# RomanBresson/KAGNN

Measured on AMD Instinct MI355X. Metric: edges/sec KAN-GIN fwd+bwd, hidden=64 grid=5, 1M-node synthetic; HBM % peak, higher is better.
Workload: dtype f32 (fp16 hi/lo split operands, fp32 accumulate)

## Files before the change

kagnn_amd/csrc/fused_calls.hip:

```cpp
#include "host.h"
#include <mutex>

using namespace kagnn;

namespace {
struct GraphSide {
    const int32_t* rowptr; const int32_t* col; const int32_t* hub_seg; int64_t num_hub_seg; int32_t hub_threshold; float self_scale;
};
struct KanChain {
    int64_t N; int32_t L; const int32_t* widths;
    const float* const* bw; const float* const* sw; const float* const* sc;
    const float* const* acts; const void* const* pack_fwd; const void* const* pack_dx;
    const float* knots; int32_t G, K, mode;
};
struct LayerIn {
    const void* x; int32_t x_dtype; int64_t ldx; const float* in_col_scale; const float* in_col_shift; float* col_mean; float* col_m2;
};
struct LayerGrads {
    const float* gy; int64_t ldgy; void* gx; int32_t gx_dtype; int64_t ldgx; int32_t bf16_gather; const float* gx_addend; int64_t ld_addend;
    float* const* g_bw; float* const* g_sw; float* const* g_sc;
};

struct GineStage {
    const float* x; int64_t ldx; const float* ea; int64_t lde; const int32_t* perm;
    float* g_ea; int64_t ldge;
    int accumulate_g_ea = 0;
    int prepacked = 0;
};
struct BnStage { const float* y; int64_t ldy; const float* weight; const float* mean; const float* rstd; float* g_weight; float* g_bias; };
struct StatsOut { const float* y; int64_t ldy; const float* mean; const float* rstd; float* sums; };
struct DwPiece { unsigned char* base; DwDefer* defer; };

struct LayerLayout {
    size_t fwd_hub_bytes, fwd_scratch, fwd_scratch_bytes, fwd_fix, fwd_fix_bytes, fwd_total;
    size_t bwd_hub_bytes, dw, dw_bytes, g[2], bwd_total;
    size_t bn, bn_ws_bytes, bn_tab, bn_bytes, stats, stats_bytes, bwd_total_all;
    size_t dw_piece[8], dw_piece_bytes[8], dw_pieces_bytes;
    int wmax;
};

void layer_layout_optional(LayerLayout& y, int64_t N, int out, int f0, int64_t num_hub_seg_t) {
    y.bn = y.bwd_total;
    y.bn_ws_bytes = out ? bn_ws_bytes(N, out) : 0;
    y.bn_tab = y.bn + al256z(y.bn_ws_bytes);
    y.bn_bytes = out ? al256z(y.bn_ws_bytes) + al256z(4 * (size_t)((out + 63) & ~63) * sizeof(float)) : 0;
    y.stats = y.bn + y.bn_bytes;
    y.stats_bytes = f0 ? al256z(bn_stats_fold_bytes(aggregate_stats_rows(N, f0, num_hub_seg_t), f0)) : 0;
    y.bwd_total_all = y.stats + y.stats_bytes;
}

int layer_layout(int64_t N, int32_t L, const int32_t* widths, int32_t G, int32_t K, int32_t mode, int64_t num_hub_seg,
                 int64_t num_hub_seg_t, LayerLayout& y) {
    static const char fn[] = "kagnn_gin_kan_layer_workspace_bytes";
    size_t fw = 0, dw = 0;
    y.wmax = 0;
    for (int l = 0; l < L; ++l) {
        int rc = check_kan_dims(fn, widths[l], widths[l + 1], G, K, mode);
        if (rc) return rc;
        size_t b = 0;
        rc = (l == L - 1 ? kagnn_kan_fwd_moments_workspace_bytes : kagnn_kan_fwd_workspace_bytes)(N, widths[l], widths[l + 1], G, K, mode, &b);
        if (rc) return rc;
        fw = b > fw ? b : fw;
        rc = kagnn_kan_bwd_weight_workspace_bytes(N, widths[l], widths[l + 1], G, K, mode, &b); if (rc) return rc;
        dw = b > dw ? b : dw;
        y.dw_piece_bytes[l] = al256z(b);
        y.wmax = widths[l] > y.wmax ? widths[l] : y.wmax;
    }
    y.dw_pieces_bytes = 0;
    for (int l = L - 1; l >= 0; --l) { y.dw_piece[l] = y.dw_pieces_bytes; y.dw_pieces_bytes += y.dw_piece_bytes[l]; }
    y.fwd_hub_bytes = al256z(aggregate_bf16_ws_bytes(num_hub_seg, widths[0]));
    y.fwd_scratch = y.fwd_hub_bytes;
    y.fwd_fix = y.fwd_scratch + al256z(fw);
    y.fwd_total = y.fwd_fix + al256z(widths[0] <= 32 ? kan_sparse_fwd_agg_ws_bytes(num_hub_seg, widths[0], widths[1]) : 0) + 256;
    y.fwd_scratch_bytes = y.fwd_total - y.fwd_scratch;
    y.fwd_fix_bytes = y.fwd_total - y.fwd_fix;
    y.bwd_hub_bytes = al256z(aggregate_bf16_ws_bytes(num_hub_seg_t, widths[0]));
    y.dw = y.bwd_hub_bytes;
    y.dw_bytes = al256z(dw);
    const size_t g_bytes = al256z((size_t)N * y.wmax * sizeof(float));
    y.g[0] = y.dw + y.dw_bytes;
    y.g[1] = y.g[0] + g_bytes;
    y.bwd_total = y.g[1] + g_bytes + 256;
    layer_layout_optional(y, N, 0, 0, 0);
    return KAGNN_OK;
}

int layer_fwd_impl(const GraphSide& gr, const KanChain& c, const LayerIn& in, const GineStage* gine, void* workspace,
                   size_t workspace_bytes, void* stream, const char* fn) {
    (void)fn;
    const int64_t N = c.N;
    const int32_t L = c.L, G = c.G, K = c.K, mode = c.mode;
    const int32_t* widths = c.widths;
    float* const* acts = const_cast<float* const*>(c.acts);
    void* const* pack_fwd = const_cast<void* const*>(c.pack_fwd);
    void* const* pack_dx = const_cast<void* const*>(c.pack_dx);
    KAGNN_CHECK_ARG(N >= 0 && L >= 1 && L <= 8 && widths && c.bw && c.sw && acts && pack_fwd && pack_dx, "bad argument");
    KAGNN_CHECK_ARG((in.in_col_scale == nullptr) == (in.in_col_shift == nullptr), "in_col_scale and in_col_shift must both be given or both be null");
    KAGNN_CHECK_ARG(!in.in_col_scale || in.x_dtype == KAGNN_DTYPE_F32, "the column affine of the gathered matrix needs fp32 rows");
    KAGNN_CHECK_ARG((in.col_mean == nullptr) == (in.col_m2 == nullptr), "col_mean and col_m2 must both be given or both be null");
    LayerLayout lay;
    int rc = layer_layout(N, L, widths, G, K, mode, gr.num_hub_seg, 0, lay);
    if (rc) return rc;
    KAGNN_CHECK_ARG(workspace && workspace_bytes >= lay.fwd_total, "workspace too small (kagnn_gin_kan_layer_workspace_bytes)");
    if (N == 0) return KAGNN_OK;
    unsigned char* ws = static_cast<unsigned char*>(workspace);
    const char* fuse_e = getenv("KAGNN_FUSE_AGG");
    const bool fuse_env = fuse_e != nullptr && atoi(fuse_e) != 0;
    const bool fuse = fuse_env && !gine && !in.in_col_scale && in.x_dtype == KAGNN_DTYPE_F32 && mode == KAGNN_PREC_SPLIT && !(L == 1 && in.col_mean) &&
                      use_sparse_fwd(widths[0], widths[1], G, K, mode) &&
                      kan_sparse_fwd_agg_ok(static_cast<const float*>(in.x), in.ldx, N, widths[0], widths[1], G, K);
    if (gine)
        rc = kagnn_aggregate_gine(static_cast<const float*>(in.x), in.ldx, gine->ea, gine->lde, acts[0], widths[0], gr.rowptr, gr.col, gine->perm, N,
                                  widths[0], gr.self_scale, stream);
    else if (fuse)
        rc = KAGNN_OK;
    else if (in.x_dtype == KAGNN_DTYPE_BF16)
        rc = kagnn_aggregate_sum_bf16(in.x, in.ldx, acts[0], widths[0], KAGNN_DTYPE_F32, gr.rowptr, gr.col, nullptr, N, widths[0], gr.self_scale,
                                      nullptr, nullptr, nullptr, 0, gr.hub_seg, gr.num_hub_seg, gr.hub_threshold, ws, lay.fwd_hub_bytes, stream);
    else if (in.in_col_scale)
        rc = kagnn_aggregate_sum_affine(static_cast<const float*>(in.x), in.ldx, acts[0], widths[0], gr.rowptr, gr.col, N, widths[0], gr.self_scale,
                                        in.in_col_scale, in.in_col_shift, gr.hub_seg, gr.num_hub_seg, gr.hub_threshold, nullptr, 0, ws,
                                        lay.fwd_hub_bytes, stream);
    else
        rc = kagnn_aggregate_sum(static_cast<const float*>(in.x), in.ldx, acts[0], widths[0], gr.rowptr, gr.col, nullptr, N, widths[0],
                                 gr.self_scale, nullptr, nullptr, nullptr, 0, gr.hub_seg, gr.num_hub_seg, gr.hub_threshold, ws, lay.fwd_hub_bytes,
                                 stream);
    if (rc) return rc;
    const bool prepacked = gine && gine->prepacked;
    bool batched = L >= 2 && !prepacked;
    int in_[8], out_[8];
    for (int l = 0; l < L; ++l) {
        in_[l] = widths[l]; out_[l] = widths[l + 1];
        batched = batched && use_split_dx(in_[l], out_[l], G, K, mode) && use_sparse_fwd(in_[l], out_[l], G, K, mode) &&
                  kan_fused_pack_ok(in_[l], out_[l], G + K);
    }
    if (batched) {
        rc = kagnn_kan_pack_batch(L, c.bw, c.sw, c.sc, in_, out_, G, K, mode, pack_fwd, pack_dx, stream);
        if (rc) return rc;
    } else if (!prepacked) {
        for (int l = 0; l < L; ++l) {
            rc = kagnn_kan_pack(c.bw[l], c.sw[l], c.sc ? c.sc[l] : nullptr, in_[l], out_[l], G, K, mode, pack_fwd[l], pack_dx[l], stream);
            if (rc) return rc;
        }
    }
    for (int l = 0; l < L; ++l) {
        if (l == 0 && fuse) {
            KAGNN_STAGE_AS("kagnn_kan_linear_fwd+aggregate_sum (one kernel)", stream);
            rc = kan_sparse_fwd_agg(static_cast<const float*>(in.x), in.ldx, N, gr.rowptr, gr.col, gr.hub_seg, gr.num_hub_seg, gr.hub_threshold,
                                    gr.self_scale, c.knots, in_[0], out_[0], G, K, pack_fwd[0], acts[0], in_[0], acts[1], out_[0],
                                    ws + lay.fwd_fix, lay.fwd_fix_bytes, as_stream(stream));
            if (rc) return rc;
            continue;
        }
        if (l == L - 1 && in.col_mean)
            rc = kagnn_kan_linear_fwd_moments(acts[l], in_[l], N, c.knots, in_[l], out_[l], G, K, mode, pack_fwd[l], acts[l + 1],
                                              out_[l], in.col_mean, in.col_m2, ws + lay.fwd_scratch, lay.fwd_scratch_bytes, stream);
        else
            rc = kagnn_kan_linear_fwd(acts[l], in_[l], N, c.knots, in_[l], out_[l], G, K, mode, pack_fwd[l], acts[l + 1], out_[l],
                                      ws + lay.fwd_scratch, lay.fwd_scratch_bytes, stream);
        if (rc) return rc;
    }
    return KAGNN_OK;
}

struct BwdSide { hipStream_t stream = nullptr; hipEvent_t fork = nullptr, join = nullptr; };
constexpr int kBwdSideMaxDevices = 64;
std::mutex g_bwd_side_mu;
BwdSide g_bwd_side[kBwdSideMaxDevices];

class BwdFork {
    std::unique_lock<std::mutex> lk_;
    BwdSide* s_ = nullptr;
    hipStream_t caller_ = nullptr;
    bool forked_ = false, recorded_ = false;
public:
    BwdFork() = default;
    BwdFork(const BwdFork&) = delete;
    BwdFork& operator=(const BwdFork&) = delete;
    int prepare(hipStream_t caller) {
        int dev = 0;
        KAGNN_HIP(hipGetDevice(&dev));
        if (dev < 0 || dev >= kBwdSideMaxDevices) return fail(KAGNN_ERR_UNSUPPORTED, "%s: device index out of range", "layer_bwd");
        lk_ = std::unique_lock<std::mutex>(g_bwd_side_mu);
        BwdSide& s = g_bwd_side[dev];
        if (!s.stream) KAGNN_HIP(hipStreamCreateWithFlags(&s.stream, hipStreamNonBlocking));
        if (!s.fork) KAGNN_HIP(hipEventCreateWithFlags(&s.fork, hipEventDisableTiming));
        if (!s.join) KAGNN_HIP(hipEventCreateWithFlags(&s.join, hipEventDisableTiming));
        s_ = &s; caller_ = caller;
        return KAGNN_OK;
    }
    int fork() {
        KAGNN_HIP(hipEventRecord(s_->fork, caller_));
        KAGNN_HIP(hipStreamWaitEvent(s_->stream, s_->fork, 0));
        forked_ = true;
        return KAGNN_OK;
    }
    hipStream_t side() const { return s_->stream; }
    int side_done(hipEvent_t* ev) {
        KAGNN_HIP(hipEventRecord(s_->join, s_->stream));
        recorded_ = true;
        *ev = s_->join;
        return KAGNN_OK;
    }
    void joined() { forked_ = false; }
    int join() {
        if (!forked_) return KAGNN_OK;
        forked_ = false;
        if (!recorded_) KAGNN_HIP(hipEventRecord(s_->join, s_->stream));
        KAGNN_HIP(hipStreamWaitEvent(caller_, s_->join, 0));
        return KAGNN_OK;
    }
    ~BwdFork() { (void)join(); }
};

constexpr int kAggCorunHeadPct = 35;
bool dw_corun_ok(int in, int out, int G, int K, int mode) {
    return use_split_dw(in, out, G, K, mode) && !g_half_products && K == 3 && G + K <= 8 && in > 32 && in <= 64 && out <= 64;
}

int layer_bwd_impl(const GraphSide& gr, const KanChain& c, const LayerGrads& io, const BnStage* bn, const float* bn_sums_in,
                   const StatsOut* so, const GineStage* gine, const DwPiece* piece, void* workspace, size_t workspace_bytes, void* stream,
                   const char* fn) {
    const int64_t N = c.N;
    const int32_t L = c.L, G = c.G, K = c.K, mode = c.mode;
    const int32_t* widths = c.widths;
    const float* const* acts = c.acts;
    void* const gx = io.gx;
    KAGNN_CHECK_ARG(N >= 0 && L >= 1 && L <= 8 && widths && c.sw && acts && c.pack_dx && io.g_sw, "bad argument");
    KAGNN_CHECK_ARG(!io.gx_addend || (gx && io.gx_dtype == KAGNN_DTYPE_F32 && !io.bf16_gather && io.ld_addend >= widths[0]),
                    "gx_addend needs an fp32 gx and fp32 gather operands");
    LayerLayout lay;
    int rc = layer_layout(N, L, widths, G, K, mode, 0, gr.num_hub_seg, lay);
    if (rc) return rc;
    layer_layout_optional(lay, N, bn ? widths[L] : 0, so ? widths[0] : 0, gr.num_hub_seg);
    KAGNN_CHECK_ARG(!so || (so->y && so->mean && so->rstd && so->sums && so->ldy >= widths[0] && gx && io.gx_dtype == KAGNN_DTYPE_F32 && !io.bf16_gather),
                    "the previous norm's statistics need its input, mean, rstd and an fp32 gx");
    KAGNN_CHECK_ARG(!bn_sums_in || bn, "bn_sums belongs to the BatchNorm stage");
    if (!(workspace && workspace_bytes >= lay.bwd_total_all))
        return fail(KAGNN_ERR_ARG, bn ? "%s: workspace too small (kagnn_gin_kan_layer_workspace_bytes + kagnn_gin_kan_layer_bwd_bn_workspace_bytes)"
                                      : "%s: workspace too small (kagnn_gin_kan_layer_workspace_bytes)", fn);
    if (N == 0) return KAGNN_OK;
    unsigned char* ws = static_cast<unsigned char*>(workspace);
    const int wmax = lay.wmax;
    unsigned char* gbuf[2] = {ws + lay.g[0], ws + lay.g[1]};
    auto dw_on = [&](void* st, int l, const float* g, long ldg) {
        unsigned char* area = piece ? piece->base + lay.dw_piece[l] : ws + lay.dw;
        const size_t bytes = piece ? lay.dw_piece_bytes[l] : lay.dw_bytes;
        return kan_linear_bwd_weight(acts[l], widths[l], nullptr, g, ldg, N, c.knots, widths[l], widths[l + 1], G, K, mode, c.sw[l],
                                     c.sc ? c.sc[l] : nullptr, io.g_bw ? io.g_bw[l] : nullptr, io.g_sw[l], io.g_sc ? io.g_sc[l] : nullptr,
                                     area, bytes, st, piece ? piece->defer : nullptr);
    };
    BwdFork side;
    struct { int l; const float* g; long ldg; } deferred[2];
    int n_deferred = 0;
    bool overlap = false;
    if (gx && !gine && !piece && !so && !io.bf16_gather && io.gx_dtype == KAGNN_DTYPE_F32 && dw_corun_ok(widths[0], widths[1], G, K, mode)) {
        const char* env = getenv("KAGNN_BWD_OVERLAP");
        const AggArgs probe{reinterpret_cast<const float*>(gbuf[0]), widths[0], static_cast<float*>(gx), io.ldgx, gr.rowptr, gr.col, nullptr, N,
                            widths[0], gr.self_scale, nullptr, nullptr, nullptr, 0, 0x7fffffff, io.gx_addend, io.ld_addend};
        const bool gx_in_ws = static_cast<unsigned char*>(gx) + (size_t)N * io.ldgx * sizeof(float) > ws &&
                              static_cast<unsigned char*>(gx) < ws + workspace_bytes;
        overlap = (env == nullptr || atoi(env) != 0) && io.ldgx >= widths[0] && (!io.gx_addend || io.ld_addend >= widths[0]) && !gx_in_ws &&
                  aggregate_corun_ok(probe);
        if (overlap) {
            hipStreamCaptureStatus cap = hipStreamCaptureStatusNone;
            if (hipStreamIsCapturing(as_stream(stream), &cap) != hipSuccess) { (void)hipGetLastError(); overlap = false; }
            else overlap = cap == hipStreamCaptureStatusNone;
        }
        if (overlap) { rc = side.prepare(as_stream(stream)); if (rc) return rc; }
    }
    auto dw = [&](int l, const float* g, long ldg) {
        const bool alive = l == 0 || (l == L - 1 && !bn);
        if (overlap && alive && dw_corun_ok(widths[l], widths[l + 1], G, K, mode)) {
            deferred[n_deferred++] = {l, g, ldg};
            return (int)KAGNN_OK;
        }
        return dw_on(stream, l, g, ldg);
    };
    const float* g = io.gy;
    long ldg = io.ldgy;
    int cur = 0;
    bool gh0_bf16 = false;
    bool bn_in_dx = false;
    BnBack bnb{};
    if (bn) {
        const int out = widths[L], ldt = (out + 63) & ~63;
        KAGNN_CHECK_ARG(bn->y && bn->mean && bn->rstd && bn->ldy >= out && N >= 2, "bad BatchNorm stage");
        unsigned char* bws = ws + lay.bn;
        float* tab = reinterpret_cast<float*>(ws + lay.bn_tab);
        bnb = BnBack{bn->y, (long)bn->ldy, tab, ldt, reinterpret_cast<float*>(gbuf[1]), (long)out};
        const int in = widths[L - 1];
        bn_in_dx = mode == KAGNN_PREC_SPLIT && use_split_dx(in, out, G, K, mode) && out <= wmax && !(L == 1 && (gx == nullptr || io.bf16_gather)) &&
                   fits32(N, ldg) && kan_split_dx_bn_ok(ldg, in, out, G, K, bnb, g);
        if (bn_in_dx && bn_sums_in) {
            KAGNN_STAGE_AS("kagnn_batchnorm_bwd statistics given (in ..._layer_bwd_bn)", stream);
            rc = bn_bwd_stats_given(bn_sums_in, N, out, bn->weight, bn->mean, bn->rstd, bn->g_weight, bn->g_bias, tab, ldt, as_stream(stream));
            if (rc) return rc;
        } else if (bn_in_dx) {
            KAGNN_STAGE_AS("kagnn_batchnorm_bwd statistics (in ..._layer_bwd_bn)", stream);
            rc = bn_bwd_stats(bn->y, bn->ldy, g, ldg, N, out, bn->weight, bn->mean, bn->rstd, bn->g_weight, bn->g_bias, tab, ldt, bws,
                              lay.bn_ws_bytes, as_stream(stream));
            if (rc) return rc;
        } else {
            if (out > wmax) return fail(KAGNN_ERR_UNSUPPORTED, "%s: a BatchNorm stage wider than every layer input is not covered", fn);
            KAGNN_STAGE_AS("kagnn_batchnorm_bwd", stream);
            rc = bn_bwd(bn->y, bn->ldy, g, ldg, N, out, bn->weight, bn->mean, bn->rstd, 1, 0.0f, 0ULL, reinterpret_cast<float*>(gbuf[1]), out,
                        bn->g_weight, bn->g_bias, bws, lay.bn_ws_bytes, as_stream(stream));
            if (rc) return rc;
            g = reinterpret_cast<const float*>(gbuf[1]); ldg = out;
        }
    }
    for (int l = L - 1; l >= 0; --l) {
        const int in = widths[l], out = widths[l + 1];
        const bool fused_bn = bn_in_dx && l == L - 1;
        if (fused_bn) {
            {
                KAGNN_STAGE_AS("kagnn_kan_linear_bwd_input", stream);
                rc = kan_split_dx_bn(acts[l], in, g, ldg, N, c.knots, in, out, G, K, c.pack_dx[l], reinterpret_cast<float*>(gbuf[0]), in, bnb,
                                     as_stream(stream));
            }
            if (rc) return rc;
            rc = dw(l, bnb.gy_out, bnb.ldo);
            if (rc) return rc;
            if (l == 0 && gx == nullptr) break;
            g = reinterpret_cast<const float*>(gbuf[0]); ldg = in; cur = 1;
            continue;
        }
        rc = dw(l, g, ldg);
        if (rc) return rc;
        if (l == 0 && gx == nullptr) break;
        const bool b16 = l == 0 && io.bf16_gather && mode == KAGNN_PREC_SPLIT && K == 3 && G + K <= 8 && out <= 128 && in % 8 == 0 &&
                         in <= 512  &&
                         use_split_dx(in, out, G, K, mode);
        rc = kagnn_kan_linear_bwd_input(acts[l], in, g, ldg, N, c.knots, in, out, G, K, mode, c.pack_dx[l], gbuf[cur], in,
                                        b16 ? KAGNN_DTYPE_BF16 : KAGNN_DTYPE_F32, stream);
        if (rc) return rc;
        g = reinterpret_cast<const float*>(gbuf[cur]); ldg = in; cur ^= 1;
        gh0_bf16 = b16;
    }
    if (gx == nullptr) return KAGNN_OK;
    const int f0 = widths[0];
    if (overlap) {
        rc = side.fork();
        if (rc) return rc;
        for (int k = 0; k < n_deferred; ++k) {
            rc = dw_on(side.side(), deferred[k].l, deferred[k].g, deferred[k].ldg);
            if (rc) return rc;
        }
        const AggArgs a{g, ldg, static_cast<float*>(gx), io.ldgx, gr.rowptr, gr.col, nullptr, N, f0, gr.self_scale, nullptr, nullptr, nullptr,
                        0, gr.hub_threshold > 0 ? gr.hub_threshold : 0x7fffffff, io.gx_addend, io.ld_addend};
        AggCorun corun{kAggCorunHeadPct * n_deferred, nullptr};
        rc = side.side_done(&corun.side_done);
        if (rc) return rc;
        KAGNN_STAGE_AS("kagnn_aggregate_sum", stream);
        rc = aggregate_sum(a, gr.hub_seg, gr.num_hub_seg, reinterpret_cast<float*>(ws), lay.bwd_hub_bytes, as_stream(stream), &corun);
        if (rc) return rc;
        side.joined();
        return KAGNN_OK;
    }
    if (gine)
        return gine_bwd(gine->x, gine->ldx, gine->ea, gine->lde, g, ldg, static_cast<float*>(gx), io.ldgx, gine->g_ea, gine->ldge,
                        gr.rowptr, gr.col, gine->perm, N, f0, gr.self_scale, as_stream(stream), gine->accumulate_g_ea);
    if (gh0_bf16 || io.gx_dtype == KAGNN_DTYPE_BF16) {
        const void* src = g;
        if (!gh0_bf16) {
            rc = kagnn_rows_to_bf16(g, ldg, gbuf[cur], f0, N, f0, stream);
            if (rc) return rc;
            src = gbuf[cur];
        }
        return kagnn_aggregate_sum_bf16(src, f0, gx, io.ldgx, io.gx_dtype, gr.rowptr, gr.col, nullptr, N, f0, gr.self_scale, nullptr, nullptr,
                                        nullptr, 0, gr.hub_seg, gr.num_hub_seg, gr.hub_threshold, ws, lay.bwd_hub_bytes, stream);
    }
    if (so) {
        AggArgs a{g, ldg, static_cast<float*>(gx), io.ldgx, gr.rowptr, gr.col, nullptr, N, f0, gr.self_scale, nullptr, nullptr, nullptr,
                  0, gr.hub_threshold > 0 ? gr.hub_threshold : 0x7fffffff, io.gx_addend, io.ld_addend};
        float* partial = reinterpret_cast<float*>(ws + lay.stats);
        a.st_y = so->y; a.st_ldy = so->ldy; a.st_mean = so->mean; a.st_rstd = so->rstd; a.st_partial = partial;
        KAGNN_CHECK_ARG(ldg >= f0 && io.ldgx >= f0 && (!io.gx_addend || io.ld_addend >= f0), "leading dimension smaller than num_feat");
        if (!aggregate_stats_ok(a)) return fail(KAGNN_ERR_UNSUPPORTED, "%s: the previous norm's statistics need 17..256 input features in 16-byte aligned fp32 rows", fn);
        {
            KAGNN_STAGE_AS("kagnn_aggregate_sum", stream);
            rc = aggregate_sum(a, gr.hub_seg, gr.num_hub_seg, reinterpret_cast<float*>(ws), lay.bwd_hub_bytes, as_stream(stream));
            if (rc) return rc;
        }
        KAGNN_STAGE_AS("kagnn_batchnorm_bwd statistics fold", stream);
        const bool hubs = gr.num_hub_seg > 0 && gr.hub_seg != nullptr && gr.hub_threshold > 0;
        return bn_sums_from_partials(partial, aggregate_stats_rows(N, f0, hubs ? gr.num_hub_seg : 0), f0, so->sums, as_stream(stream));
    }
    return kagnn_aggregate_sum_add(g, ldg, static_cast<float*>(gx), io.ldgx, gr.rowptr, gr.col, nullptr, N, f0, gr.self_scale, nullptr,
                                   nullptr, nullptr, 0, gr.hub_seg, gr.num_hub_seg, gr.hub_threshold, io.gx_addend, io.ld_addend, ws,
                                   lay.bwd_hub_bytes, stream);
}

struct StackLayout {
    LayerLayout layer;
    size_t fwd_layer_bytes, bn_ws, bn_ws_bytes, moments, fwd_total;
    size_t bwd_layer_bytes, pp[2], arena, arena_conv_bytes, arena_bytes, bwd_total;
};

int stack_layout(int64_t N, int32_t nconv, int32_t L, const int32_t* widths, int32_t G, int32_t K, int32_t mode, StackLayout& s) {
    int rc = layer_layout(N, L, widths, G, K, mode, 0, 0, s.layer);
    if (rc) return rc;
    layer_layout_optional(s.layer, N, widths[L], 0, 0);
    s.fwd_layer_bytes = al256z(s.layer.fwd_total);
    s.bn_ws = s.fwd_layer_bytes;
    s.bn_ws_bytes = bn_ws_bytes(N, widths[L]);
    s.moments = s.bn_ws + al256z(s.bn_ws_bytes);
    s.fwd_total = s.moments + al256z(2 * (size_t)widths[L] * sizeof(float)) + 256;
    s.bwd_layer_bytes = al256z(s.layer.bwd_total_all);
    const size_t g_bytes = al256z((size_t)N * widths[0] * sizeof(float));
    s.pp[0] = s.bwd_layer_bytes;
    s.pp[1] = s.pp[0] + g_bytes;
    s.arena = s.pp[1] + g_bytes;
    s.arena_conv_bytes = nconv * L <= kDwDeferMax ? s.layer.dw_pieces_bytes : 0;
    s.arena_bytes = s.arena_conv_bytes * (size_t)nconv;
    s.bwd_total = s.arena + s.arena_bytes + 256;
    return KAGNN_OK;
}

int stack_fwd_impl(const float* x, int64_t ldx, const float* edge_attr, int64_t lde, int64_t N, const int32_t* rowptr,
                   const int32_t* col, const int32_t* perm, const float* self_scale, int32_t nconv,
                   int32_t L, const int32_t* widths, const float* const* bw, const float* const* sw,
                   const float* const* sc, const float* knots, int32_t G, int32_t K, int32_t mode,
                   float* const* acts, void* const* pack_fwd, void* const* pack_dx,
                   const float* const* bn_weight, const float* const* bn_bias, float* const* running_mean,
                   float* const* running_var, const float* momentum, const float* eps,
                   float* const* h, float* const* save_mean, float* const* save_rstd,
                   void* workspace, size_t workspace_bytes, void* stream, bool prepacked) {
    static const char fn[] = "kagnn_gine_kan_stack_fwd";
    ModeScope mode_scope_(mode);
    KAGNN_CHECK_ARG_AS(fn, nconv >= 1 && L >= 1 && L <= 8 && widths && self_scale && bw && sw && acts && pack_fwd && pack_dx && bn_weight && bn_bias &&
                       momentum && eps && h && save_mean && save_rstd, "null array");
    KAGNN_CHECK_ARG_AS(fn, widths[0] == widths[L] && N >= 2, "hidden -> hidden chains, at least two rows (batch statistics)");
    StackLayout lay;
    int rc = stack_layout(N, nconv, L, widths, G, K, mode, lay);
    if (rc) return rc;
    KAGNN_CHECK_ARG_AS(fn, workspace && workspace_bytes >= lay.fwd_total, "workspace too small (kagnn_gine_kan_stack_workspace_bytes)");
    unsigned char* ws = static_cast<unsigned char*>(workspace);
    float* mom = reinterpret_cast<float*>(ws + lay.moments);
    const int H = widths[L];
    int in_[16], out_[16];
    bool batch = nconv * L <= 16;
    for (int k = 0; k < nconv * L && batch; ++k) {
        in_[k] = widths[k % L]; out_[k] = widths[k % L + 1];
        batch = use_split_dx(in_[k], out_[k], G, K, mode) && use_sparse_fwd(in_[k], out_[k], G, K, mode) && kan_fused_pack_ok(in_[k], out_[k], G + K);
    }
    if (batch && !prepacked) { rc = kagnn_kan_pack_batch(nconv * L, bw, sw, sc, in_, out_, G, K, mode, pack_fwd, pack_dx, stream); if (rc) return rc; }
    const float* in = x;
    int64_t ldin = ldx;
    for (int i = 0; i < nconv; ++i) {
        GineStage gs{in, ldin, edge_attr, lde, perm, nullptr, 0};
        gs.prepacked = batch ? 1 : 0;
        const GraphSide gr{.rowptr = rowptr, .col = col, .self_scale = self_scale[i]};
        const KanChain c{.N = N, .L = L, .widths = widths, .bw = bw + i * L, .sw = sw + i * L, .sc = sc ? sc + i * L : nullptr,
                         .acts = acts + i * (L + 1), .pack_fwd = pack_fwd + i * L, .pack_dx = pack_dx + i * L, .knots = knots, .G = G, .K = K,
                         .mode = mode};
        const LayerIn li{.x = in, .x_dtype = KAGNN_DTYPE_F32, .ldx = ldin, .col_mean = mom,
                         .col_m2 = mom + H};
        rc = layer_fwd_impl(gr, c, li, &gs, ws, lay.fwd_layer_bytes, stream, fn);
        if (rc) return rc;
        rc = kagnn_batchnorm_fwd(acts[i * (L + 1) + L], H, N, H, bn_weight[i], bn_bias[i], running_mean ? running_mean[i] : nullptr,
                                 running_var ? running_var[i] : nullptr, momentum[i], eps[i], 1, mom, mom + H, 0.0f, 0ULL, h[i], H,
                                 save_mean[i], save_rstd[i], ws + lay.bn_ws, lay.bn_ws_bytes, stream);
        if (rc) return rc;
        in = h[i]; ldin = H;
    }
    return KAGNN_OK;
}
}

#pragma GCC visibility push(default)
extern "C" {

int kagnn_gin_kan_layer_workspace_bytes(int64_t N, int32_t L, const int32_t* widths, int32_t G, int32_t K, int32_t mode,
                                        int64_t num_hub_seg, int64_t num_hub_seg_t, size_t* fwd_bytes, size_t* bwd_bytes) {
    ModeScope mode_scope_(mode);
    KAGNN_CHECK_ARG(N >= 0 && L >= 1 && L <= 8 && widths && fwd_bytes && bwd_bytes, "bad argument");
    LayerLayout lay;
    int rc = layer_layout(N, L, widths, G, K, mode, num_hub_seg, num_hub_seg_t, lay);
    if (rc) return rc;
    *fwd_bytes = lay.fwd_total;
    *bwd_bytes = lay.bwd_total;
    return KAGNN_OK;
}

int kagnn_gin_kan_layer_fwd(const void* x, int32_t x_dtype, int64_t ldx, int64_t N, const int32_t* rowptr, const int32_t* col,
                            const int32_t* hub_seg, int64_t num_hub_seg, int32_t hub_threshold, float self_scale,
                            int32_t L, const int32_t* widths, const float* const* bw, const float* const* sw,
                            const float* const* sc, const float* knots, int32_t G, int32_t K, int32_t mode,
                            float* const* acts, void* const* pack_fwd, void* const* pack_dx, float* col_mean,
                            float* col_m2, void* workspace, size_t workspace_bytes, void* stream) {
    ModeScope mode_scope_(mode);
    const GraphSide gr{.rowptr = rowptr, .col = col, .hub_seg = hub_seg, .num_hub_seg = num_hub_seg, .hub_threshold = hub_threshold,
                       .self_scale = self_scale};
    const KanChain c{.N = N, .L = L, .widths = widths, .bw = bw, .sw = sw, .sc = sc, .acts = acts, .pack_fwd = pack_fwd, .pack_dx = pack_dx,
                     .knots = knots, .G = G, .K = K, .mode = mode};
    const LayerIn in{.x = x, .x_dtype = x_dtype, .ldx = ldx, .col_mean = col_mean, .col_m2 = col_m2};
    return layer_fwd_impl(gr, c, in, nullptr, workspace, workspace_bytes, stream, __func__);
}

int kagnn_gin_kan_layer_fwd_affine(const float* x, int64_t ldx, int64_t N, const int32_t* rowptr, const int32_t* col,
                                   const int32_t* hub_seg, int64_t num_hub_seg, int32_t hub_threshold, float self_scale,
                                   const float* in_col_scale, const float* in_col_shift,
                                   int32_t L, const int32_t* widths, const float* const* bw, const float* const* sw,
                                   const float* const* sc, const float* knots, int32_t G, int32_t K, int32_t mode,
                                   float* const* acts, void* const* pack_fwd, void* const* pack_dx, float* col_mean,
                                   float* col_m2, void* workspace, size_t workspace_bytes, void* stream) {
    ModeScope mode_scope_(mode);
    const GraphSide gr{.rowptr = rowptr, .col = col, .hub_seg = hub_seg, .num_hub_seg = num_hub_seg, .hub_threshold = hub_threshold,
                       .self_scale = self_scale};
    const KanChain c{.N = N, .L = L, .widths = widths, .bw = bw, .sw = sw, .sc = sc, .acts = acts, .pack_fwd = pack_fwd, .pack_dx = pack_dx,
                     .knots = knots, .G = G, .K = K, .mode = mode};
    const LayerIn in{.x = x, .x_dtype = KAGNN_DTYPE_F32, .ldx = ldx, .in_col_scale = in_col_scale, .in_col_shift = in_col_shift,
                     .col_mean = col_mean, .col_m2 = col_m2};
    return layer_fwd_impl(gr, c, in, nullptr, workspace, workspace_bytes, stream, __func__);
}

int kagnn_gin_kan_layer_bwd_add(const float* gy, int64_t ldgy, int64_t N, const int32_t* rowptr_t, const int32_t* col_t,
                                const int32_t* hub_seg_t, int64_t num_hub_seg_t, int32_t hub_threshold, float self_scale,
                                int32_t L, const int32_t* widths, const float* const* sw, const float* const* sc,
                                const float* knots, int32_t G, int32_t K, int32_t mode, const float* const* acts,
                                const void* const* pack_dx, void* gx, int32_t gx_dtype, int64_t ldgx, int32_t bf16_gather,
                                const float* gx_addend, int64_t ld_addend,
                                float* const* g_bw, float* const* g_sw, float* const* g_sc, void* workspace,
                                size_t workspace_bytes, void* stream) {
    ModeScope mode_scope_(mode);
    const GraphSide gr{.rowptr = rowptr_t, .col = col_t, .hub_seg = hub_seg_t, .num_hub_seg = num_hub_seg_t, .hub_threshold = hub_threshold,
                       .self_scale = self_scale};
    const KanChain c{.N = N, .L = L, .widths = widths, .sw = sw, .sc = sc, .acts = acts, .pack_dx = pack_dx,
                     .knots = knots, .G = G, .K = K, .mode = mode};
    const LayerGrads io{.gy = gy, .ldgy = ldgy, .gx = gx, .gx_dtype = gx_dtype, .ldgx = ldgx, .bf16_gather = bf16_gather, .gx_addend = gx_addend,
                        .ld_addend = ld_addend, .g_bw = g_bw, .g_sw = g_sw, .g_sc = g_sc};
    return layer_bwd_impl(gr, c, io, nullptr, nullptr, nullptr, nullptr, nullptr, workspace, workspace_bytes, stream, __func__);
}

int kagnn_gin_kan_layer_bwd_bn_workspace_bytes(int64_t N, int32_t out, size_t* bytes) {
    KAGNN_CHECK_ARG(N >= 0 && out >= 1 && bytes, "bad argument");
    LayerLayout lay{};
    layer_layout_optional(lay, N, out, 0, 0);
    *bytes = lay.bn_bytes;
    return KAGNN_OK;
}

int kagnn_gin_kan_layer_bwd_bn(const float* g, int64_t ldg, const float* y, int64_t ldy, const float* bn_weight,
                               const float* bn_mean, const float* bn_rstd, float* g_bn_weight, float* g_bn_bias,
                               int64_t N, const int32_t* rowptr_t, const int32_t* col_t,
                               const int32_t* hub_seg_t, int64_t num_hub_seg_t, int32_t hub_threshold, float self_scale,
                               int32_t L, const int32_t* widths, const float* const* sw, const float* const* sc,
                               const float* knots, int32_t G, int32_t K, int32_t mode, const float* const* acts,
                               const void* const* pack_dx, void* gx, int32_t gx_dtype, int64_t ldgx, int32_t bf16_gather,
                               const float* gx_addend, int64_t ld_addend,
                               float* const* g_bw, float* const* g_sw, float* const* g_sc, void* workspace,
                               size_t workspace_bytes, void* stream) {
    ModeScope mode_scope_(mode);
    const BnStage bn{y, ldy, bn_weight, bn_mean, bn_rstd, g_bn_weight, g_bn_bias};
    const GraphSide gr{.rowptr = rowptr_t, .col = col_t, .hub_seg = hub_seg_t, .num_hub_seg = num_hub_seg_t, .hub_threshold = hub_threshold,
                       .self_scale = self_scale};
    const KanChain c{.N = N, .L = L, .widths = widths, .sw = sw, .sc = sc, .acts = acts, .pack_dx = pack_dx,
                     .knots = knots, .G = G, .K = K, .mode = mode};
    const LayerGrads io{.gy = g, .ldgy = ldg, .gx = gx, .gx_dtype = gx_dtype, .ldgx = ldgx, .bf16_gather = bf16_gather, .gx_addend = gx_addend,
                        .ld_addend = ld_addend, .g_bw = g_bw, .g_sw = g_sw, .g_sc = g_sc};
    return layer_bwd_impl(gr, c, io, &bn, nullptr, nullptr, nullptr, nullptr, workspace, workspace_bytes, stream, __func__);
}

int kagnn_gin_kan_layer_bwd_bn_sums_workspace_bytes(int64_t N, int32_t in_features, int64_t num_hub_seg_t, size_t* bytes) {
    KAGNN_CHECK_ARG(N >= 0 && in_features >= 1 && num_hub_seg_t >= 0 && bytes, "bad argument");
    LayerLayout lay{};
    layer_layout_optional(lay, N, 0, in_features, num_hub_seg_t);
    *bytes = lay.stats_bytes;
    return KAGNN_OK;
}

int kagnn_gin_kan_layer_bwd_bn_sums(const float* g, int64_t ldg, const float* y, int64_t ldy, const float* bn_weight,
                                    const float* bn_mean, const float* bn_rstd, float* g_bn_weight, float* g_bn_bias,
                                    const float* bn_sums,
                                    const float* prev_y, int64_t ld_prev_y, const float* prev_mean, const float* prev_rstd,
                                    float* prev_sums,
                                    int64_t N, const int32_t* rowptr_t, const int32_t* col_t,
                                    const int32_t* hub_seg_t, int64_t num_hub_seg_t, int32_t hub_threshold, float self_scale,
                                    int32_t L, const int32_t* widths, const float* const* sw, const float* const* sc,
                                    const float* knots, int32_t G, int32_t K, int32_t mode, const float* const* acts,
                                    const void* const* pack_dx, void* gx, int32_t gx_dtype, int64_t ldgx, int32_t bf16_gather,
                                    const float* gx_addend, int64_t ld_addend,
                                    float* const* g_bw, float* const* g_sw, float* const* g_sc, void* workspace,
                                    size_t workspace_bytes, void* stream) {
    ModeScope mode_scope_(mode);
    const BnStage bn{y, ldy, bn_weight, bn_mean, bn_rstd, g_bn_weight, g_bn_bias};
    const StatsOut so{prev_y, ld_prev_y, prev_mean, prev_rstd, prev_sums};
    KAGNN_CHECK_ARG((prev_sums == nullptr) == (prev_y == nullptr), "prev_y and prev_sums come together");
    const GraphSide gr{.rowptr = rowptr_t, .col = col_t, .hub_seg = hub_seg_t, .num_hub_seg = num_hub_seg_t, .hub_threshold = hub_threshold,
                       .self_scale = self_scale};
    const KanChain c{.N = N, .L = L, .widths = widths, .sw = sw, .sc = sc, .acts = acts, .pack_dx = pack_dx,
                     .knots = knots, .G = G, .K = K, .mode = mode};
    const LayerGrads io{.gy = g, .ldgy = ldg, .gx = gx, .gx_dtype = gx_dtype, .ldgx = ldgx, .bf16_gather = bf16_gather, .gx_addend = gx_addend,
                        .ld_addend = ld_addend, .g_bw = g_bw, .g_sw = g_sw, .g_sc = g_sc};
    return layer_bwd_impl(gr, c, io, &bn, bn_sums, prev_sums ? &so : nullptr, nullptr, nullptr, workspace, workspace_bytes, stream, __func__);
}

int kagnn_gin_kan_layer_bwd(const float* gy, int64_t ldgy, int64_t N, const int32_t* rowptr_t, const int32_t* col_t,
                            const int32_t* hub_seg_t, int64_t num_hub_seg_t, int32_t hub_threshold, float self_scale,
                            int32_t L, const int32_t* widths, const float* const* sw, const float* const* sc,
                            const float* knots, int32_t G, int32_t K, int32_t mode, const float* const* acts,
                            const void* const* pack_dx, void* gx, int32_t gx_dtype, int64_t ldgx, int32_t bf16_gather,
                            float* const* g_bw, float* const* g_sw, float* const* g_sc, void* workspace,
                            size_t workspace_bytes, void* stream) {
    ModeScope mode_scope_(mode);
    return kagnn_gin_kan_layer_bwd_add(gy, ldgy, N, rowptr_t, col_t, hub_seg_t, num_hub_seg_t, hub_threshold, self_scale, L, widths, sw,
                                       sc, knots, G, K, mode, acts, pack_dx, gx, gx_dtype, ldgx, bf16_gather, nullptr, 0, g_bw, g_sw,
                                       g_sc, workspace, workspace_bytes, stream);
}

int kagnn_gine_kan_layer_fwd(const float* x, int64_t ldx, const float* edge_attr, int64_t lde, int64_t N, const int32_t* rowptr,
                             const int32_t* col, const int32_t* perm, float self_scale,
                             int32_t L, const int32_t* widths, const float* const* bw, const float* const* sw,
                             const float* const* sc, const float* knots, int32_t G, int32_t K, int32_t mode,
                             float* const* acts, void* const* pack_fwd, void* const* pack_dx, float* col_mean,
                             float* col_m2, void* workspace, size_t workspace_bytes, void* stream) {
    ModeScope mode_scope_(mode);
    KAGNN_CHECK_ARG(N == 0 || (x && edge_attr && perm && widths && ldx >= widths[0] && lde >= widths[0]), "null array or short leading dimension");
    const GineStage gs{x, ldx, edge_attr, lde, perm, nullptr, 0};
    const GraphSide gr{.rowptr = rowptr, .col = col, .self_scale = self_scale};
    const KanChain c{.N = N, .L = L, .widths = widths, .bw = bw, .sw = sw, .sc = sc, .acts = acts, .pack_fwd = pack_fwd, .pack_dx = pack_dx,
                     .knots = knots, .G = G, .K = K, .mode = mode};
    const LayerIn in{.x = x, .x_dtype = KAGNN_DTYPE_F32, .ldx = ldx, .col_mean = col_mean,
                     .col_m2 = col_m2};
    return layer_fwd_impl(gr, c, in, &gs, workspace, workspace_bytes, stream, __func__);
}

int kagnn_gine_kan_layer_bwd(const float* g, int64_t ldg, const float* bn_y, int64_t ld_bn_y, const float* bn_weight,
                             const float* bn_mean, const float* bn_rstd, float* g_bn_weight, float* g_bn_bias,
                             const float* x, int64_t ldx, const float* edge_attr, int64_t lde, int64_t N,
                             const int32_t* rowptr_t, const int32_t* col_t, const int32_t* perm_t, float self_scale,
                             int32_t L, const int32_t* widths, const float* const* sw, const float* const* sc,
                             const float* knots, int32_t G, int32_t K, int32_t mode, const float* const* acts,
                             const void* const* pack_dx, float* gx, int64_t ldgx, float* g_edge_attr, int64_t ldge,
                             float* const* g_bw, float* const* g_sw, float* const* g_sc, void* workspace,
                             size_t workspace_bytes, void* stream) {
    ModeScope mode_scope_(mode);
    KAGNN_CHECK_ARG(N == 0 || (x && edge_attr && perm_t && gx && widths && ldx >= widths[0] && lde >= widths[0] && ldgx >= widths[0]),
                    "null array or short leading dimension (gx is required: the edge-attribute gradient comes out of the same kernel)");
    KAGNN_CHECK_ARG(!g_edge_attr || ldge >= widths[0], "short leading dimension of g_edge_attr");
    const GineStage gs{x, ldx, edge_attr, lde, perm_t, g_edge_attr, ldge};
    const BnStage bn{bn_y, ld_bn_y, bn_weight, bn_mean, bn_rstd, g_bn_weight, g_bn_bias};
    const GraphSide gr{.rowptr = rowptr_t, .col = col_t, .self_scale = self_scale};
    const KanChain c{.N = N, .L = L, .widths = widths, .sw = sw, .sc = sc, .acts = acts, .pack_dx = pack_dx,
                     .knots = knots, .G = G, .K = K, .mode = mode};
    const LayerGrads io{.gy = g, .ldgy = ldg, .gx = gx, .gx_dtype = KAGNN_DTYPE_F32, .ldgx = ldgx, .g_bw = g_bw, .g_sw = g_sw, .g_sc = g_sc};
    return layer_bwd_impl(gr, c, io, bn_y ? &bn : nullptr, nullptr, nullptr, &gs, nullptr, workspace, workspace_bytes, stream, __func__);
}

int kagnn_gine_kan_stack_workspace_bytes(int64_t N, int32_t nconv, int32_t L, const int32_t* widths, int32_t G, int32_t K, int32_t mode,
                                         size_t* fwd_bytes, size_t* bwd_bytes) {
    ModeScope mode_scope_(mode);
    KAGNN_CHECK_ARG(N >= 0 && nconv >= 1 && L >= 1 && L <= 8 && widths && fwd_bytes && bwd_bytes, "bad argument");
    KAGNN_CHECK_ARG(widths[0] == widths[L], "every convolution of the stack maps hidden -> hidden");
    StackLayout lay;
    int rc = stack_layout(N, nconv, L, widths, G, K, mode, lay);
    if (rc) return rc;
    *fwd_bytes = lay.fwd_total;
    *bwd_bytes = lay.bwd_total;
    return KAGNN_OK;
// ... 355 lines not shown
```

Before: 4.482 billion.

## Overlap weight packing with forward aggregation and fork backward side stream earlier

```diff
diff --git a/kagnn_amd/csrc/fused_calls.hip b/kagnn_amd/csrc/fused_calls.hip
--- a/kagnn_amd/csrc/fused_calls.hip
+++ b/kagnn_amd/csrc/fused_calls.hip
@@ -31,6 +31,71 @@
 struct StatsOut { const float* y; int64_t ldy; const float* mean; const float* rstd; float* sums; };
 struct DwPiece { unsigned char* base; DwDefer* defer; };
 
+struct SideStream { hipStream_t stream = nullptr; hipEvent_t fork = nullptr, join = nullptr; };
+constexpr int kSideMaxDevices = 64;
+std::mutex g_side_mu;
+SideStream g_side[kSideMaxDevices];
+
+class SideFork {
+    std::unique_lock<std::mutex> lk_;
+    SideStream* s_ = nullptr;
+    hipStream_t caller_ = nullptr;
+    bool forked_ = false;
+public:
+    SideFork() = default;
+    SideFork(const SideFork&) = delete;
+    SideFork& operator=(const SideFork&) = delete;
+    int prepare(hipStream_t caller) {
+        int dev = 0;
+        KAGNN_HIP(hipGetDevice(&dev));
+        if (dev < 0 || dev >= kSideMaxDevices) return fail(KAGNN_ERR_UNSUPPORTED, "%s: device index out of range", "layer call");
+        lk_ = std::unique_lock<std::mutex>(g_side_mu);
+        SideStream& s = g_side[dev];
+        if (!s.stream) KAGNN_HIP(hipStreamCreateWithFlags(&s.stream, hipStreamNonBlocking));
+        if (!s.fork) KAGNN_HIP(hipEventCreateWithFlags(&s.fork, hipEventDisableTiming));
+        if (!s.join) KAGNN_HIP(hipEventCreateWithFlags(&s.join, hipEventDisableTiming));
+        s_ = &s; caller_ = caller;
+        return KAGNN_OK;
+    }
+    int fork() {
+        KAGNN_HIP(hipEventRecord(s_->fork, caller_));
+        KAGNN_HIP(hipStreamWaitEvent(s_->stream, s_->fork, 0));
+        forked_ = true;
+        return KAGNN_OK;
+    }
+    bool forked() const { return forked_; }
+    hipStream_t side() const { return s_->stream; }
+    int side_mark(hipEvent_t* ev) {
+        KAGNN_HIP(hipEventRecord(s_->join, s_->stream));
+        *ev = s_->join;
+        return KAGNN_OK;
+    }
+    int join() {
+        if (!forked_) return KAGNN_OK;
+        forked_ = false;
+        KAGNN_HIP(hipEventRecord(s_->join, s_->stream));
+        KAGNN_HIP(hipStreamWaitEvent(caller_, s_->join, 0));
+        return KAGNN_OK;
+    }
+    ~SideFork() { (void)join(); }
+};
+
+bool stream_not_capturing(void* stream) {
+    hipStreamCaptureStatus cap = hipStreamCaptureStatusNone;
+    if (hipStreamIsCapturing(as_stream(stream), &cap) != hipSuccess) { (void)hipGetLastError(); return false; }
+    return cap == hipStreamCaptureStatusNone;
+}
+bool env_on(const char* name) {
+    const char* env = getenv(name);
+    return env == nullptr || atoi(env) != 0;
+}
+
+constexpr int kAggCorunHeadPct = 27;
+constexpr bool kForkBeforeLastDx = true;
+bool dw_corun_ok(int in, int out, int G, int K, int mode) {
+    return use_split_dw(in, out, G, K, mode) && !g_half_products && K == 3 && G + K <= 8 && in > 32 && in <= 64 && out <= 64;
+}
+
 struct LayerLayout {
     size_t fwd_hub_bytes, fwd_scratch, fwd_scratch_bytes, fwd_fix, fwd_fix_bytes, fwd_total;
     size_t bwd_hub_bytes, dw, dw_bytes, g[2], bwd_total;
@@ -109,6 +174,32 @@
     const bool fuse = fuse_env && !gine && !in.in_col_scale && in.x_dtype == KAGNN_DTYPE_F32 && mode == KAGNN_PREC_SPLIT && !(L == 1 && in.col_mean) &&
                       use_sparse_fwd(widths[0], widths[1], G, K, mode) &&
                       kan_sparse_fwd_agg_ok(static_cast<const float*>(in.x), in.ldx, N, widths[0], widths[1], G, K);
+    const bool prepacked = gine && gine->prepacked;
+    bool batched = L >= 2 && !prepacked;
+    int in_[8], out_[8];
+    for (int l = 0; l < L; ++l) {
+        in_[l] = widths[l]; out_[l] = widths[l + 1];
+        batched = batched && use_split_dx(in_[l], out_[l], G, K, mode) && use_sparse_fwd(in_[l], out_[l], G, K, mode) &&
+                  kan_fused_pack_ok(in_[l], out_[l], G + K);
+    }
+    auto packs_on = [&](void* st) {
+        if (batched) return kagnn_kan_pack_batch(L, c.bw, c.sw, c.sc, in_, out_, G, K, mode, pack_fwd, pack_dx, st);
+        for (int l = 0; l < L && !prepacked; ++l) {
+            const int prc = kagnn_kan_pack(c.bw[l], c.sw[l], c.sc ? c.sc[l] : nullptr, in_[l], out_[l], G, K, mode, pack_fwd[l], pack_dx[l], st);
+            if (prc) return prc;
+        }
+        return (int)KAGNN_OK;
+    };
+    SideFork side;
+    if (!gine && !fuse && mode == KAGNN_PREC_SPLIT && !g_half_products && env_on("KAGNN_FWD_OVERLAP") && stream_not_capturing(stream)) {
+        rc = side.prepare(as_stream(stream));
+        if (rc) return rc;
+        rc = side.fork();
+        if (rc) return rc;
+        rc = packs_on(side.side());
+        if (rc) return rc;
+    }
+    const bool packs_aside = side.forked();
     if (gine)
         rc = kagnn_aggregate_gine(static_cast<const float*>(in.x), in.ldx, gine->ea, gine->lde, acts[0], widths[0], gr.rowptr, gr.col, gine->perm, N,
                                   widths[0], gr.self_scale, stream);
@@ -126,23 +217,8 @@
                                  gr.self_scale, nullptr, nullptr, nullptr, 0, gr.hub_seg, gr.num_hub_seg, gr.hub_threshold, ws, lay.fwd_hub_bytes,
                                  stream);
     if (rc) return rc;
-    const bool prepacked = gine && gine->prepacked;
-    bool batched = L >= 2 && !prepacked;
-    int in_[8], out_[8];
-    for (int l = 0; l < L; ++l) {
-        in_[l] = widths[l]; out_[l] = widths[l + 1];
-        batched = batched && use_split_dx(in_[l], out_[l], G, K, mode) && use_sparse_fwd(in_[l], out_[l], G, K, mode) &&
-                  kan_fused_pack_ok(in_[l], out_[l], G + K);
-    }
-    if (batched) {
-        rc = kagnn_kan_pack_batch(L, c.bw, c.sw, c.sc, in_, out_, G, K, mode, pack_fwd, pack_dx, stream);
-        if (rc) return rc;
-    } else if (!prepacked) {
-        for (int l = 0; l < L; ++l) {
-            rc = kagnn_kan_pack(c.bw[l], c.sw[l], c.sc ? c.sc[l] : nullptr, in_[l], out_[l], G, K, mode, pack_fwd[l], pack_dx[l], stream);
-            if (rc) return rc;
-        }
-    }
+    rc = packs_aside ? side.join() : packs_on(stream);
+    if (rc) return rc;
     for (int l = 0; l < L; ++l) {
         if (l == 0 && fuse) {
             KAGNN_STAGE_AS("kagnn_kan_linear_fwd+aggregate_sum (one kernel)", stream);
@@ -161,61 +237,6 @@
         if (rc) return rc;
     }
     return KAGNN_OK;
-}
-
-struct BwdSide { hipStream_t stream = nullptr; hipEvent_t fork = nullptr, join = nullptr; };
-constexpr int kBwdSideMaxDevices = 64;
-std::mutex g_bwd_side_mu;
-BwdSide g_bwd_side[kBwdSideMaxDevices];
-
-class BwdFork {
-    std::unique_lock<std::mutex> lk_;
-    BwdSide* s_ = nullptr;
-    hipStream_t caller_ = nullptr;
-    bool forked_ = false, recorded_ = false;
-public:
-    BwdFork() = default;
-    BwdFork(const BwdFork&) = delete;
-    BwdFork& operator=(const BwdFork&) = delete;
-    int prepare(hipStream_t caller) {
-        int dev = 0;
-        KAGNN_HIP(hipGetDevice(&dev));
-        if (dev < 0 || dev >= kBwdSideMaxDevices) return fail(KAGNN_ERR_UNSUPPORTED, "%s: device index out of range", "layer_bwd");
-        lk_ = std::unique_lock<std::mutex>(g_bwd_side_mu);
-        BwdSide& s = g_bwd_side[dev];
-        if (!s.stream) KAGNN_HIP(hipStreamCreateWithFlags(&s.stream, hipStreamNonBlocking));
-        if (!s.fork) KAGNN_HIP(hipEventCreateWithFlags(&s.fork, hipEventDisableTiming));
-        if (!s.join) KAGNN_HIP(hipEventCreateWithFlags(&s.join, hipEventDisableTiming));
-        s_ = &s; caller_ = caller;
-        return KAGNN_OK;
-    }
-    int fork() {
-        KAGNN_HIP(hipEventRecord(s_->fork, caller_));
-        KAGNN_HIP(hipStreamWaitEvent(s_->stream, s_->fork, 0));
-        forked_ = true;
-        return KAGNN_OK;
-    }
-    hipStream_t side() const { return s_->stream; }
-    int side_done(hipEvent_t* ev) {
-        KAGNN_HIP(hipEventRecord(s_->join, s_->stream));
-        recorded_ = true;
-        *ev = s_->join;
-        return KAGNN_OK;
-    }
-    void joined() { forked_ = false; }
-    int join() {
-        if (!forked_) return KAGNN_OK;
-        forked_ = false;
-        if (!recorded_) KAGNN_HIP(hipEventRecord(s_->join, s_->stream));
-        KAGNN_HIP(hipStreamWaitEvent(caller_, s_->join, 0));
-        return KAGNN_OK;
-    }
-    ~BwdFork() { (void)join(); }
-};
-
-constexpr int kAggCorunHeadPct = 35;
-bool dw_corun_ok(int in, int out, int G, int K, int mode) {
-    return use_split_dw(in, out, G, K, mode) && !g_half_products && K == 3 && G + K <= 8 && in > 32 && in <= 64 && out <= 64;
 }
 
 int layer_bwd_impl(const GraphSide& gr, const KanChain& c, const LayerGrads& io, const BnStage* bn, const float* bn_sums_in,
@@ -243,30 +264,25 @@
     unsigned char* ws = static_cast<unsigned char*>(workspace);
     const int wmax = lay.wmax;
     unsigned char* gbuf[2] = {ws + lay.g[0], ws + lay.g[1]};
-    auto dw_on = [&](void* st, int l, const float* g, long ldg) {
+    DwDefer side_defer{};
+    auto dw_on = [&](void* st, int l, const float* g, long ldg, bool aside) {
         unsigned char* area = piece ? piece->base + lay.dw_piece[l] : ws + lay.dw;
         const size_t bytes = piece ? lay.dw_piece_bytes[l] : lay.dw_bytes;
         return kan_linear_bwd_weight(acts[l], widths[l], nullptr, g, ldg, N, c.knots, widths[l], widths[l + 1], G, K, mode, c.sw[l],
                                      c.sc ? c.sc[l] : nullptr, io.g_bw ? io.g_bw[l] : nullptr, io.g_sw[l], io.g_sc ? io.g_sc[l] : nullptr,
-                                     area, bytes, st, piece ? piece->defer : nullptr);
+                                     area, bytes, st, piece ? piece->defer : aside ? &side_defer : nullptr);
     };
-    BwdFork side;
+    SideFork side;
     struct { int l; const float* g; long ldg; } deferred[2];
     int n_deferred = 0;
     bool overlap = false;
     if (gx && !gine && !piece && !so && !io.bf16_gather && io.gx_dtype == KAGNN_DTYPE_F32 && dw_corun_ok(widths[0], widths[1], G, K, mode)) {
-        const char* env = getenv("KAGNN_BWD_OVERLAP");
         const AggArgs probe{reinterpret_cast<const float*>(gbuf[0]), widths[0], static_cast<float*>(gx), io.ldgx, gr.rowptr, gr.col, nullptr, N,
                             widths[0], gr.self_scale, nullptr, nullptr, nullptr, 0, 0x7fffffff, io.gx_addend, io.ld_addend};
         const bool gx_in_ws = static_cast<unsigned char*>(gx) + (size_t)N * io.ldgx * sizeof(float) > ws &&
                               static_cast<unsigned char*>(gx) < ws + workspace_bytes;
-        overlap = (env == nullptr || atoi(env) != 0) && io.ldgx >= widths[0] && (!io.gx_addend || io.ld_addend >= widths[0]) && !gx_in_ws &&
-                  aggregate_corun_ok(probe);
-        if (overlap) {
-            hipStreamCaptureStatus cap = hipStreamCaptureStatusNone;
-            if (hipStreamIsCapturing(as_stream(stream), &cap) != hipSuccess) { (void)hipGetLastError(); overlap = false; }
-            else overlap = cap == hipStreamCaptureStatusNone;
-        }
+        overlap = env_on("KAGNN_BWD_OVERLAP") && io.ldgx >= widths[0] && (!io.gx_addend || io.ld_addend >= widths[0]) && !gx_in_ws &&
+                  aggregate_corun_ok(probe) && stream_not_capturing(stream);
         if (overlap) { rc = side.prepare(as_stream(stream)); if (rc) return rc; }
     }
     auto dw = [&](int l, const float* g, long ldg) {
@@ -275,7 +291,16 @@
             deferred[n_deferred++] = {l, g, ldg};
             return (int)KAGNN_OK;
         }
-        return dw_on(stream, l, g, ldg);
+        return dw_on(stream, l, g, ldg, false);
+    };
+    hipEvent_t corun_mark = nullptr;
+    auto fork_side = [&]() {
+        int frc = side.fork();
+        for (int k = 0; k < n_deferred && !frc; ++k) {
+            if (k == 1) frc = dw_defer_flush(&side_defer, side.side());
+            if (!frc) frc = dw_on(side.side(), deferred[k].l, deferred[k].g, deferred[k].ldg, true);
+        }
+        return frc ? frc : side.side_mark(&corun_mark);
     };
     const float* g = io.gy;
     long ldg = io.ldgy;
@@ -329,6 +354,7 @@
         rc = dw(l, g, ldg);
         if (rc) return rc;
         if (l == 0 && gx == nullptr) break;
+        if (kForkBeforeLastDx && overlap && l == 0 && L >= 2) { rc = fork_side(); if (rc) return rc; }
         const bool b16 = l == 0 && io.bf16_gather && mode == KAGNN_PREC_SPLIT && K == 3 && G + K <= 8 && out <= 128 && in % 8 == 0 &&
                          in <= 512  &&
                          use_split_dx(in, out, G, K, mode);
@@ -341,22 +367,18 @@
     if (gx == nullptr) return KAGNN_OK;
     const int f0 = widths[0];
     if (overlap) {
-        rc = side.fork();
-        if (rc) return rc;
-        for (int k = 0; k < n_deferred; ++k) {
-            rc = dw_on(side.side(), deferred[k].l, deferred[k].g, deferred[k].ldg);
-            if (rc) return rc;
-        }
+        if (!side.forked()) { rc = fork_side(); if (rc) return rc; }
         const AggArgs a{g, ldg, static_cast<float*>(gx), io.ldgx, gr.rowptr, gr.col, nullptr, N, f0, gr.self_scale, nullptr, nullptr, nullptr,
                         0, gr.hub_threshold > 0 ? gr.hub_threshold : 0x7fffffff, io.gx_addend, io.ld_addend};
-        AggCorun corun{kAggCorunHeadPct * n_deferred, nullptr};
-        rc = side.side_done(&corun.side_done);
-        if (rc) return rc;
-        KAGNN_STAGE_AS("kagnn_aggregate_sum", stream);
-        rc = aggregate_sum(a, gr.hub_seg, gr.num_hub_seg, reinterpret_cast<float*>(ws), lay.bwd_hub_bytes, as_stream(stream), &corun);
-        if (rc) return rc;
-        side.joined();
-        return KAGNN_OK;
+        const AggCorun corun{kAggCorunHeadPct * n_deferred, corun_mark};
+        {
+            KAGNN_STAGE_AS("kagnn_aggregate_sum", stream);
+            rc = aggregate_sum(a, gr.hub_seg, gr.num_hub_seg, reinterpret_cast<float*>(ws), lay.bwd_hub_bytes, as_stream(stream), &corun);
+            if (rc) return rc;
+        }
+        rc = dw_defer_flush(&side_defer, side.side());
+        if (rc) return rc;
+        return side.join();
     }
     if (gine)
         return gine_bwd(gine->x, gine->ldx, gine->ea, gine->lde, g, ldg, static_cast<float*>(gx), io.ldgx, gine->g_ea, gine->ldge,
```

After: 4.492 billion, median of 2. No clear change (+0.2%).
